# kakaoenterprise/JORLDY

Hardware: NVIDIA H100
Metric: env_steps_per_sec (higher is better)
Workload: dtype f32

## Files before the change

include/jorldy_b200.h:

```cpp
#ifndef JORLDY_B200_H
#define JORLDY_B200_H

#include <stdint.h>

#ifdef __cplusplus
#define JB_API extern "C"
#else
#define JB_API
#endif

JB_API int jb_env_classic_reset(int kind, double* phys, float* obs, int32_t* elapsed, int64_t* episode,
                                float* score, const uint8_t* mask, uint64_t seed, uint64_t stream_base,
                                int n, void* stream);
JB_API int jb_env_classic_step(int kind, double* phys, float* obs, int32_t* elapsed, int64_t* episode,
                               float* score, const void* action, int action_kind, float* next_obs,
                               float* reward, float* done, float* stats, int auto_reset, int max_steps,
                               uint64_t seed, uint64_t stream_base, int n, void* stream);

JB_API int jb_gae(const float* reward, const float* done, const float* value, const float* next_value,
                  const float* last_value, int N, int T, float gamma, float lambda, int standardize,
                  float* adv, float* ret, void* stream);

JB_API int
jb_env_synth_reset(float* obs, int32_t* elapsed, int64_t* episode, float* score, uint64_t seed,
// ... 59 lines not shown
JB_API int jb_heads_bwd_dw(const float* dout, const float* h, int M, int H, float* dw0, float* db0, int n0, float* dw1,
                           float* db1, int n1, float* dw2, float* db2, int n2, void* stream);
JB_API int jb_heads_fwd_n(const float* h, int M, int H, int n_heads, const float* const* w, const float* const* b,
                          const int* n, float* out, void* stream);
JB_API int jb_heads_bwd_dx_n(const float* dout, const float* h, int M, int H, int n_heads, const float* const* w,
                             const int* n, float* dh, void* stream);
JB_API int jb_heads_bwd_dw_n(const float* dout, const float* h, int M, int H, int n_heads, float* const* dw,
                             float* const* db, const int* n, void* stream);

JB_API int jb_ppo_act_discrete(const float* out, int M, int A, int nout, const float* u, uint64_t seed,
                               uint64_t stream_base, uint64_t ctr, long long* row_ctr, int greedy, int64_t* action,
                               void* stream);
JB_API int jb_ppo_act_continuous(const float* out, int M, int A, int nout, const float* normal, uint64_t seed,
                                 uint64_t stream_base, uint64_t ctr, long long* row_ctr, int greedy, float* action,
                                 void* stream);
JB_API int jb_ppo_prepass_discrete(const float* out, const int32_t* action, int M, int A, int nout, float* value,
                                   float* logp_old, void* stream);
JB_API int jb_ppo_prepass_continuous(const float* out, const float* action, int M, int A, int nout, float* value,
                                     float* logp_old, void* stream);
JB_API int jb_take_minibatch(const int32_t* perm, long long* cursor, int B, int32_t* cur_idx, void* stream);
JB_API int jb_ppo_loss(int continuous, const float* out, const int32_t* idx, const void* action, const float* adv,
                       const float* ret, const float* value_old, const float* logp_old, int B, int A, int nout,
                       float eps_clip, float vf_coef, float ent_coef, float* dout, float* stats, float* acc,
                       void* stream);

JB_API int jb_vmpo_loss(int continuous, const float* out, const float* out_old, const int32_t* idx, const void* action,
                        const float* adv, const float* ret, int B, int A, int nout, const float* mult, float eps_eta,
                        float eps_alpha_mu, float eps_alpha_sigma, float* dout, float* dmult, float* stats, float* acc,
                        void* stream);
JB_API int jb_vmpo_clamp(float* mult, float min_eta, float min_alpha_mu, float min_alpha_sigma, void* stream);
// ... 161 lines not shown
```

jorldy_b200/core/agent/ppo.py:

```python
import numpy as np
import torch

from ..buffer import FrameRollout, RolloutBuffer
from ..dev import C, ptr, require_cuda, stream_ptr
from ..network import Network
from ..optimizer import Optimizer
from .base import BaseAgent

GRAPH_CHUNK = 16
MAX_ACTION_SIZE = {"discrete": 18, "continuous": 8}


class PPO(BaseAgent):
    def __init__(
        self,
        state_size,
        action_size,
        hidden_size=512,
        network="discrete_policy_value",
        head="mlp",
        optim_config={"name": "adam"},
        gamma=0.99,
        use_standardization=True,
        run_step=1e6,
# ... 50 lines not shown
        self.use_fused = use_fused
        self._fused = {}
        self._graphs = {}
        self._acc = torch.zeros(8, dtype=torch.float32, device=self.device)
        self._cursor = torch.zeros(1, dtype=torch.int64, device=self.device)
        self.world_size = 1
        self.allreduce = None
        self._inject_perms = None
        self.n_launches = 0
        self.n_prepass_launches = 0

    @property
    def continuous(self):
        return self.action_type == "continuous"

    def act_device(self, state, training=True, noise=None):
        net = self.network
        M = state.shape[0]
        out = net._buf("act.out", (M, net.nout))
        net.forward_rows(state, out)
        A = self.action_size
        row_ctr = self._row_counter(M)
        if self.continuous:
            action = net._buf("act.a", (M, A))
            C.jb_ppo_act_continuous(ptr(out), M, A, net.nout, ptr(noise), self.seed, self.rng_stream_base,
                                    0, ptr(row_ctr), int(not training), ptr(action), stream_ptr())
        else:
            action = net._buf("act.a", (M,), torch.int64)
            C.jb_ppo_act_discrete(ptr(out), M, A, net.nout, ptr(noise), self.seed, self.rng_stream_base,
                                  0, ptr(row_ctr), int(not training), ptr(action), stream_ptr())
        return action

    @torch.no_grad()
    def act(self, state, training=True):
        self.network.train(training)
        s = self.as_tensor(state)
        action = self.act_device(s.view(s.shape[0], -1), training)
        a = action.cpu().numpy()
        return {"action": a.reshape(a.shape[0], -1)}

    def _minibatch_step(self, st, idx, B):
        net = self.network
        tag = f"mb{B}."
        out = net.forward_raw(st["state"], idx, B, tag=tag)
        dout = net._buf(tag + "dout", (B, net.nout))
# ... 43 lines not shown
            dst.copy_(src)
        graph = torch.cuda.CUDAGraph()
        with torch.cuda.graph(graph):
            chunk()
        self._graphs[key] = graph
        return graph

    def _gae_reward(self, st, reward, next_state, N, T):
        return reward

    def _advantages(self, st, state, action, reward, done, next_state, last_next_state, next_rows, N, T):
        net = self.network
        NT = N * T
        A = self.action_size
        s = stream_ptr()
        net.forward_rows(state, st["out"])
        if self.continuous:
            C.jb_ppo_prepass_continuous(ptr(st["out"]), ptr(action), NT, A, net.nout, ptr(st["value"]),
                                        ptr(st["logp_old"]), s)
        else:
            C.jb_ppo_prepass_discrete(ptr(st["out"]), ptr(action), NT, A, net.nout, ptr(st["value"]),
                                      ptr(st["logp_old"]), s)
        if next_state is not None:
            nout = net._buf("next.out", (NT, net.nout))
            net.forward_rows(next_state, nout)
            st["next_value"].copy_(nout[:, -1])
            nv, lv = st["next_value"], None
        else:
            lout = net._buf("last.out", (N, net.nout))
            net.forward_rows(last_next_state, lout)
            lv = net._buf("last.v", (N,))
            lv.copy_(lout[:, -1])
            nv = None
        reward = self._gae_reward(st, reward, next_state if next_state is not None else next_rows, N, T)
        C.jb_gae(ptr(reward), ptr(done), ptr(st["value"]), ptr(nv), ptr(lv), N, T, self.gamma, self._lambda,
                 int(self.use_standardization), ptr(st["adv"]), ptr(st["ret"]), s)
        return st["ret"].mean()

    def _learn_tensors(self, state, action, reward, done, next_state=None, last_next_state=None, next_rows=None):
        net = self.network
        NT = state.shape[0]
        T = self.n_step
        N = NT // T
        assert N * T == NT, f"rollout of {NT} rows is not a multiple of n_step={T} (ppo.py:97 view(-1, n_step) would raise)"
        A = self.action_size
        dev = self.device
        st = getattr(self, "_st", None)
        if st is None or st["NT"] != NT:
            st = {"NT": NT,
                  "out": torch.empty(NT, net.nout, device=dev),
                  "value": torch.empty(NT, device=dev),
                  "logp_old": torch.empty(NT, A if self.continuous else 1, device=dev),
                  "adv": torch.empty(NT, device=dev), "ret": torch.empty(NT, device=dev),
                  "next_value": torch.empty(NT, device=dev),
                  "perm": torch.empty(NT, dtype=torch.int32, device=dev)}
            self._st = st
        st["state"] = state
        st["action"] = action
        mean_ret = self._advantages(st, state, action, reward, done, next_state, last_next_state, next_rows, N, T)

        B = self.batch_size
        self._begin_epochs()
        n_full = NT // B
        tail = NT - n_full * B
        from . import ppo_fused
        use_fused = self.use_fused and n_full > 0 and ppo_fused.supported(self, B)
        if use_fused and B not in self._fused:
            self._fused[B] = ppo_fused.FusedRunner(self, B)
        use_graph = (not use_fused) and self.use_cuda_graph and n_full >= GRAPH_CHUNK
        n_steps = 0
        for epoch in range(self.n_epoch):
            if self._inject_perms is not None:
                perm = torch.as_tensor(np.asarray(self._inject_perms[epoch]), dtype=torch.int32, device=dev)
# ... 5 lines not shown
            if use_fused:
                self._fused[B].run(st, n_full)
                done_steps = n_full
            if use_graph:
                g = self._graph_for(st, B)
                for _ in range(n_full // GRAPH_CHUNK):
                    g.replay()
                done_steps = (n_full // GRAPH_CHUNK) * GRAPH_CHUNK
            for k in range(done_steps, n_full):
                self._minibatch_step(st, st["perm"][k * B:(k + 1) * B], B)
            if tail:
                self._minibatch_step(st, st["perm"][n_full * B:], tail)
            n_steps += n_full + (1 if tail else 0)
        self.n_launches = (self.n_epoch * (1 + (self.LAUNCHES_PER_MINIBATCH if tail else 0)) if use_fused
                           else n_steps * self.LAUNCHES_PER_MINIBATCH)
        n_chunks = (NT + 16383) // 16384
        self.n_prepass_launches = 3 * n_chunks + 1 + 3 + 1
        return self._learn_result(mean_ret)

    def _learn_result(self, mean_ret):
        acc = torch.cat([self._acc[:6], mean_ret.view(1), self._acc[7:8]]).cpu().numpy()
        if acc[7] != 0.0:
            dbg = [ws["partials"][200:205].tolist() for ws in (r.ws for r in self._fused.values())]
            raise RuntimeError("persistent PPO kernel: a peer GPU did not reach the gradient exchange (flag wait timed out); "
                               f"[kind 1=grad-ready 2=done-reading, peer, step, seen, target] = {dbg}")
        cnt = max(acc[5], 1.0)
        return {
            "actor_loss": float(acc[0] / cnt),
            "critic_loss": float(acc[1] / cnt),
            "entropy_loss": float(acc[2] / cnt),
            "max_ratio": float(acc[3]),
# ... 25 lines not shown
        hin["next_state"].copy_(torch.as_tensor(tr["next_state"], dtype=torch.float32, device=dev).reshape(n, -1))
        hin["reward"].copy_(torch.as_tensor(tr["reward"], dtype=torch.float32, device=dev).reshape(-1))
        hin["done"].copy_(torch.as_tensor(tr["done"], dtype=torch.float32, device=dev).reshape(-1))
        hin["action"].copy_(self._action_to_device(tr["action"]))
        return self._learn_tensors(hin["state"], hin["action"], hin["reward"], hin["done"], next_state=hin["next_state"])

    def learn_rollout(self, rollout):
        N, T = rollout.N, rollout.T
        frames = isinstance(rollout, FrameRollout)
        if frames:
            state, last = rollout.rows(), rollout.last_rows()
        else:
            state, last = rollout.state.view(N * T, -1), rollout.last_next_state
        res = self._learn_tensors(state, rollout.action.view(N * T, -1) if self.continuous
                                  else rollout.action.view(N * T), rollout.reward.view(N * T),
                                  rollout.done.view(N * T), last_next_state=last, next_rows=rollout.next_rows())
        if frames:
            rollout.frames.check()
        rollout.clear()
        return res

    def process(self, transitions, step):
        result = {}
        self.memory.store(transitions)
        delta_t = step - self.time_t
        self.time_t = step
        self.learn_stamp += delta_t
        if self.learn_stamp >= self.n_step:
            result = self.learn()
            if self.lr_decay:
                self.learning_rate_decay(step)
# ... 3 lines not shown
```

jorldy_b200/core/agent/rnd_ppo.py:

```python
import os

import numpy as np
import torch

from ..dev import C, ptr, stream_ptr
from ..network.policy_value import ContinuousPolicyTwoValue, DiscretePolicyTwoValue
from ..network.rnd import FEATURE, RND
from ..optimizer import Optimizer
from .base import cpu_state_dict
from .curiosity import _RunningMeanStd, check_batch_norm_rows, load_two_adam_state, two_adam_state
from .ppo import MAX_ACTION_SIZE, PPO

RND_NETWORKS = {"rnd_mlp": "mlp", "rnd_cnn": "cnn"}
TWO_VALUE_NETWORKS = {"discrete_policy_value": DiscretePolicyTwoValue, "continuous_policy_value": ContinuousPolicyTwoValue}


class RND_PPO(PPO):
    _GRAPH_INPUTS = PPO._GRAPH_INPUTS + ("value_i", "ret_i", "rnd_next", "rnd_target")
    replicas_only = True
    FAMILY = "RND-PPO"
    needs_next_state = True

    def __init__(self, state_size, action_size, optim_config={"name": "adam"}, rnd_network="rnd_mlp", gamma_i=0.99,
                 extrinsic_coeff=2.0, intrinsic_coeff=1.0, obs_normalize=True, ri_normalize=True, batch_norm=True,
# ... 62 lines not shown

    def _advantages(self, st, state, action, reward, done, next_state, last_next_state, next_rows, N, T):
        net = self.network
        NT = N * T
        s = stream_ptr()
        self._check_batch(NT)
        s_next = next_state if next_state is not None else next_rows
        if s_next is None:
            raise ValueError("RND-PPO needs every step's next state (a rollout with next_state, or host transitions)")
        st["rnd_next"] = s_next
        ri = self._intrinsic_reward(s_next, N, T)
        st["rnd_target"] = self.rnd.target_cache(NT)
        self._ri_mean = ri.mean()
        buf = lambda k: net._buf("rnd." + k, (NT,))
        st["value_i"], st["ret_i"] = buf("value_i"), buf("ret_i")
        net.forward_rows(state, st["out"])
        C.jb_rnd_prepass(int(self.continuous), ptr(st["out"]), ptr(action), NT, self.action_size, net.nout,
                         ptr(st["value"]), ptr(st["value_i"]), ptr(st["logp_old"]), s)
        nout = net._buf("next.out", (NT, net.nout))
        net.forward_rows(s_next, nout)
        st["next_value"].copy_(nout[:, -2])
        nv_i = buf("next_value_i")
        nv_i.copy_(nout[:, -1])
        adv_e, adv_i = buf("adv_e"), buf("adv_i")
        C.jb_gae(ptr(reward), ptr(done), ptr(st["value"]), ptr(st["next_value"]), 0, N, T, self.gamma, self._lambda, 0,
                 ptr(adv_e), ptr(st["ret"]), s)
        if self.non_episodic:
            done_i = buf("no_done")
            done_i.zero_()
        else:
# ... 75 lines not shown
```

jorldy_b200/core/buffer/rollout_buffer.py:

```python
import numpy as np
import torch

from ..dev import require_cuda
from .base import BaseBuffer
from .frame_store import FrameRows, FrameStore, frames_per_rollout


class RolloutBuffer(BaseBuffer):
    def __init__(self):
        super().__init__()
        self.buffer = list()

    def store(self, transitions):
        if self.first_store:
            self.check_dim(transitions[0])
        self.buffer += transitions

    def sample(self):
        transitions = self.stack_transition(self.buffer)
        self.buffer.clear()
        return transitions

    def sample_batched(self):
        out = {}
        for key in self.buffer[0].keys():
            arr = np.stack([np.asarray(b[key]) for b in self.buffer], axis=1)
            out[key] = arr.reshape((-1,) + arr.shape[2:])
        self.buffer.clear()
        return out

    @property
    def size(self):
        return len(self.buffer)


class DeviceRollout:

    def __init__(self, num_envs, n_step, state_size, action_size, action_type, device=None, next_state=False):
        dev = require_cuda(device)
        N, T = num_envs, n_step
        self.N, self.T, self.device = N, T, dev
        self.state = torch.zeros(N, T, state_size, dtype=torch.float32, device=dev)
        if action_type == "discrete":
            self.action = torch.zeros(N, T, dtype=torch.int32, device=dev)
        else:
            self.action = torch.zeros(N, T, action_size, dtype=torch.float32, device=dev)
        self.reward = torch.zeros(N, T, dtype=torch.float32, device=dev)
        self.done = torch.zeros(N, T, dtype=torch.float32, device=dev)
        self.last_next_state = torch.zeros(N, state_size, dtype=torch.float32, device=dev)
        self.next_state = torch.zeros(N, T, state_size, dtype=torch.float32, device=dev) if next_state else None
        self.t = 0

    def next_rows(self):
        return None if self.next_state is None else self.next_state.view(self.N * self.T, -1)

    def write(self, state, action, reward, done, next_state):
        t = self.t
        self.state[:, t].copy_(state)
        if self.action.dtype == torch.int32:
            self.action[:, t].copy_(action.view(self.N))
        else:
            self.action[:, t].copy_(action.view(self.N, -1))
        self.reward[:, t].copy_(reward)
        self.done[:, t].copy_(done)
        if self.next_state is not None:
            self.next_state[:, t].copy_(next_state)
        if t == self.T - 1:
            self.last_next_state.copy_(next_state)
        self.t = t + 1

    def write_after_step(self, action, reward, done, next_state):
        t = self.t
        if self.action.dtype == torch.int32:
            self.action[:, t].copy_(action.view(self.N))
        else:
            self.action[:, t].copy_(action.view(self.N, -1))
        self.reward[:, t].copy_(reward)
        self.done[:, t].copy_(done)
        if self.next_state is not None:
            self.next_state[:, t].copy_(next_state)
        if t == self.T - 1:
            self.last_next_state.copy_(next_state)
        self.t = t + 1

    @property
    def full(self):
        return self.t >= self.T

    def clear(self):
        self.t = 0

# ... 2 lines not shown

    def __init__(self, num_envs, n_step, action_size, action_type, device=None, next_state=False):
        dev = require_cuda(device)
        N, T = num_envs, n_step
        self.N, self.T, self.device = N, T, dev
        self.frames = FrameStore(N, frames_per_rollout(T), dev)
        self.state_ref = torch.zeros(N, T, dtype=torch.int64, device=dev)
        if action_type == "discrete":
            self.action = torch.zeros(N, T, dtype=torch.int32, device=dev)
        else:
            self.action = torch.zeros(N, T, action_size, dtype=torch.float32, device=dev)
        self.reward = torch.zeros(N, T, dtype=torch.float32, device=dev)
        self.done = torch.zeros(N, T, dtype=torch.float32, device=dev)
        self.last_next_state = torch.zeros(N, dtype=torch.int64, device=dev)
        self.next_state = None
        self.next_ref = torch.zeros(N, T, dtype=torch.int64, device=dev) if next_state else None
        self._refs = torch.zeros(2, N, dtype=torch.int64, device=dev)
        self.t = 0

    def start(self, obs):
        self.frames.start(obs)

    def push(self, obs, next_obs, done, auto_reset):
        s, x = self.frames.push(obs, next_obs, done, auto_reset, out=self._refs)
        self.state_ref[:, self.t].copy_(s)
        if self.next_ref is not None:
            self.next_ref[:, self.t].copy_(x)
        return x

    def rows(self):
# ... 8 lines not shown
```

jorldy_b200/core/collect.py:

```python
import torch

from .buffer import DeviceRollout, FrameRollout, frame_store


class RolloutCollector:
    def __init__(self, env, agent, n_step=None, use_cuda_graph=True):
        self.env, self.agent = env, agent
        self.T = n_step or agent.n_step
        self.frames = bool(getattr(env, "frame_stack", False))
        if self.frames:
            self.rollout = FrameRollout(env.num_envs, self.T, env.action_size, env.action_type, device=agent.device,
                                        next_state=getattr(agent, "needs_next_state", False))
        else:
            self.rollout = DeviceRollout(env.num_envs, self.T, env.state_size, env.action_size, env.action_type,
                                         device=agent.device, next_state=getattr(agent, "needs_next_state", False))
        self.use_cuda_graph = use_cuda_graph
        self._graph = None
        self.launches_per_collect = 5 * self.T
        env.reset_device()
        if self.frames:
            self.rollout.start(env.obs)

    def _collect_eager(self):
        env, agent, ro = self.env, self.agent, self.rollout
        ro.clear()
        for t in range(self.T):
            if not self.frames:
                ro.state[:, t].copy_(env.obs)
            action = agent.act_device(env.obs, training=True)
            next_obs, reward, done = env.step_device(action)
            ro.t = t
            if self.frames:
                next_obs = ro.push(env.obs, next_obs, done, env.auto_reset)
            ro.write_after_step(action, reward, done, next_obs)

    def collect(self):
        if not self.use_cuda_graph:
            self._collect_eager()
            return self.rollout
        if self._graph is None:
            side = torch.cuda.Stream()
            side.wait_stream(torch.cuda.current_stream())
            with torch.cuda.stream(side):
                self._collect_eager()
            torch.cuda.current_stream().wait_stream(side)
            torch.cuda.synchronize()
            g = torch.cuda.CUDAGraph()
            with torch.cuda.graph(g):
                self._collect_eager()
# ... 139 lines not shown
```

jorldy_b200/core/network/layers.py:

```python
from ..dev import C, ptr, stream_ptr


import ctypes
import os

TC_MIN_ROWS = 1024
_USE_TC = os.environ.get("JB_NO_TC", "0") != "1"


def linear_fwd(x, w, b, y, relu):
    M, in_f = x.shape
    out_f = w.shape[0]
    if _USE_TC and M >= TC_MIN_ROWS and M % 128 == 0 and out_f % 128 == 0 and in_f % 32 == 0 and b is not None:
        C.jb_linear_fwd_tc(ptr(x), ptr(w), ptr(b), ptr(y), M, in_f, out_f, int(relu), stream_ptr())
        return
    C.jb_linear_fwd(ptr(x), ptr(w), ptr(b), ptr(y), M, in_f, out_f, int(relu), stream_ptr())


def linear_bwd_dx(dy, w, dx, relu_act=None, accumulate=False):
    M, out_f = dy.shape
    in_f = w.shape[1]
    if accumulate:
        C.jb_gemm(ptr(dy), out_f, 1, ptr(w), in_f, 0, ptr(dx), in_f, M, in_f, out_f, 0, 0,
                  ptr(relu_act), in_f, 0, 1, stream_ptr())
# ... 25 lines not shown
    M, out_f = dy.shape
    C.jb_linear_io_bwd_dw(ptr(dy), ptr(x), ptr(dw), M, x.shape[1], out_f, stream_ptr())
    C.jb_colsum(ptr(dy), M, out_f, ptr(db), 0, stream_ptr())


def _ptrs(ts, kind=ctypes.c_void_p):
    return (kind * len(ts))(*ts)


def heads_fwd(h, heads, out):
    M, H = h.shape
    C.jb_heads_fwd_n(ptr(h), M, H, len(heads), _ptrs([ptr(w) for w, _ in heads]), _ptrs([ptr(b) for _, b in heads]),
                     _ptrs([w.shape[0] for w, _ in heads], ctypes.c_int), ptr(out), stream_ptr())


def heads_bwd_dx(dout, h, heads, dh):
    M, H = h.shape
    C.jb_heads_bwd_dx_n(ptr(dout), ptr(h), M, H, len(heads), _ptrs([ptr(w) for w, _ in heads]),
                        _ptrs([w.shape[0] for w, _ in heads], ctypes.c_int), ptr(dh), stream_ptr())


def heads_bwd_dw(dout, h, grads):
    M, H = h.shape
    C.jb_heads_bwd_dw_n(ptr(dout), ptr(h), M, H, len(grads), _ptrs([ptr(dw) for dw, _ in grads]),
                        _ptrs([ptr(db) for _, db in grads]), _ptrs([dw.shape[0] for dw, _ in grads], ctypes.c_int),
                        stream_ptr())
```

jorldy_b200/core/network/policy_value.py:

```python
import torch

from .base import FlatNetwork, init_gain, orthogonal_
from .head import make_head
from . import layers as L


class _PolicyValue(FlatNetwork):
    head_names = ()

    def __init__(self, D_in, D_out, D_hidden=512, head="mlp", device=None, seed=None):
        super().__init__(device)
        self.D_in, self.D_out, self.D_hidden = D_in, D_out, D_hidden
        self.head = make_head(head, D_in, D_hidden)
        self.out_heads = self._out_heads(D_out)
        self.nout = sum(n for _, n, _ in self.out_heads)
        self._wide = self.nout > 32
        assert not self._wide or len(self.out_heads) == 1
        specs = self.head.specs() + [("l.weight", (D_hidden, self.head.D_head_out)), ("l.bias", (D_hidden,))]
        for name, n, _ in self.out_heads:
            specs += [(f"{name}.weight", (n, D_hidden)), (f"{name}.bias", (n,))]
        self._specs = specs
        self._allocate()
        gen = torch.Generator().manual_seed(seed) if seed is not None else None
        with torch.no_grad():
            self.head.init(self.p, gen)
            self.p["l.weight"].copy_(orthogonal_((D_hidden, self.head.D_head_out), init_gain("relu"), gen))
            for name, n, gain in self.out_heads:
                self.p[f"{name}.weight"].copy_(orthogonal_((n, D_hidden), init_gain(gain), gen))

    def _heads_wb(self):
        return [(self.p[f"{n}.weight"], self.p[f"{n}.bias"]) for n, _, _ in self.out_heads]

    def _heads_grads(self):
        return [(self.g[f"{n}.weight"], self.g[f"{n}.bias"]) for n, _, _ in self.out_heads]

    def forward_raw(self, x, idx=None, M=None, out=None, tag="t.", save=True):
        M = M if M is not None else (idx.shape[0] if idx is not None else x.shape[0])
        h1 = self.head.forward(self, x, idx, M, tag, save)
        h2 = self._buf(tag + "h2", (M, self.D_hidden))
        L.linear_fwd(h1, self.p["l.weight"], self.p["l.bias"], h2, relu=True)
        if out is None:
            out = self._buf(tag + "out", (M, self.nout))
        if self._wide:
            w, b = self._heads_wb()[0]
            L.linear_fwd(h2, w, b, out, relu=False)
        else:
            L.heads_fwd(h2, self._heads_wb(), out)
        return out

    def forward_rows(self, x, out):
        M = x.shape[0]
        for s in range(0, M, self.head.max_rows):
            e = min(M, s + self.head.max_rows)
            self.forward_raw(x[s:e], None, e - s, out[s:e], tag=f"inf{e - s}.", save=False)
        return out

    def backward_raw(self, dout, M, tag="t."):
        h1 = self._buf(tag + "head.h", (M, self.head.D_head_out))
        h2 = self._buf(tag + "h2", (M, self.D_hidden))
        dh2 = self._buf(tag + "dh2", (M, self.D_hidden))
        dh1 = self._buf(tag + "dh1", (M, self.head.D_head_out))
        if self._wide:
            (w, _), (dw, db) = self._heads_wb()[0], self._heads_grads()[0]
            L.linear_bwd_dw(dout, h2, dw, db)
            L.linear_bwd_dx(dout, w, dh2, relu_act=h2)
        else:
            L.heads_bwd_dw(dout, h2, self._heads_grads())
            L.heads_bwd_dx(dout, h2, self._heads_wb(), dh2)
        L.linear_bwd_dw(dh2, h1, self.g["l.weight"], self.g["l.bias"])
# ... 37 lines not shown
```

jorldy_b200/csrc/heads.cu:

```cuda
#include "common.cuh"

namespace {

constexpr int MAX_DIN = 32;
constexpr int MAX_NOUT = 32;

__global__ void mlp_in_fwd_kernel(const float* __restrict__ x, const int32_t* __restrict__ idx,
                                  const float* __restrict__ W1, const float* __restrict__ b1,
                                  int M, int D, int H, float* __restrict__ h1, float* __restrict__ xg) {
  const int m = blockIdx.y;
  const int j = blockIdx.x * blockDim.x + threadIdx.x;
  __shared__ float sx[MAX_DIN];
  const int row = idx ? idx[m] : m;
  if (threadIdx.x < D) {
    const float v = x[(size_t)row * D + threadIdx.x];
    sx[threadIdx.x] = v;
    if (xg && blockIdx.x == 0) xg[(size_t)m * D + threadIdx.x] = v;
  }
  __syncthreads();
  if (j >= H) return;
  float acc = 0.f;
  for (int i = 0; i < D; ++i) acc = fmaf(sx[i], W1[(size_t)j * D + i], acc);
  acc += b1[j];
  h1[(size_t)m * H + j] = fmaxf(acc, 0.f);
}

struct HeadRows {
  const float* w[MAX_NOUT];
  const float* b[MAX_NOUT];
};
struct HeadGradRows {
  float* dw[MAX_NOUT];
  float* db[MAX_NOUT];
};

__global__ void __launch_bounds__(256)
heads_fwd_kernel(const float* __restrict__ h, int M, int H, HeadRows hr, int nout, float* __restrict__ out) {
  const int warp = (blockIdx.x * blockDim.x + threadIdx.x) >> 5;
  const int lane = threadIdx.x & 31;
  if (warp >= M) return;
  float acc[MAX_NOUT];
#pragma unroll
  for (int o = 0; o < MAX_NOUT; ++o) acc[o] = 0.f;
  const float* hrow = h + (size_t)warp * H;
  int j = lane;
  for (; j + 96 < H; j += 128) {
    float hv[4];
#pragma unroll
    for (int u = 0; u < 4; ++u) hv[u] = hrow[j + 32 * u];
#pragma unroll
    for (int o = 0; o < MAX_NOUT; ++o) {
      if (o < nout) {
        float wv[4];
#pragma unroll
        for (int u = 0; u < 4; ++u) wv[u] = hr.w[o][j + 32 * u];
#pragma unroll
        for (int u = 0; u < 4; ++u) acc[o] = fmaf(hv[u], wv[u], acc[o]);
      }
    }
  }
  for (; j < H; j += 32) {
    const float hv = hrow[j];
#pragma unroll
    for (int o = 0; o < MAX_NOUT; ++o)
      if (o < nout) acc[o] = fmaf(hv, hr.w[o][j], acc[o]);
  }
#pragma unroll
  for (int o = 0; o < MAX_NOUT; ++o) {
    if (o < nout) {
      const float v = jb_warp_sum(acc[o]);
      if (lane == 0) out[(size_t)warp * nout + o] = v + *hr.b[o];
    }
  }
}

__global__ void heads_bwd_dx_kernel(const float* __restrict__ dout, const float* __restrict__ h, int M, int H,
                                    HeadRows hr, int nout, float* __restrict__ dh) {
  const int m = blockIdx.y;
  const int j = blockIdx.x * blockDim.x + threadIdx.x;
  __shared__ float sd[MAX_NOUT];
  if (threadIdx.x < nout) sd[threadIdx.x] = dout[(size_t)m * nout + threadIdx.x];
  __syncthreads();
  if (j >= H) return;
  float acc = 0.f;
#pragma unroll
  for (int o = 0; o < MAX_NOUT; ++o)
    if (o < nout) acc = fmaf(sd[o], hr.w[o][j], acc);
  dh[(size_t)m * H + j] = (h[(size_t)m * H + j] > 0.f) ? acc : 0.f;
// ... 44 lines not shown
    float v = bacc;
#pragma unroll
    for (int q = 0; q < MAX_NOUT; ++q) if (q == o && o < nout) v = acc[q];
    __syncthreads();
    s[ry][threadIdx.x] = v;
    __syncthreads();
    if (ry == 0) {
      float t = s[0][threadIdx.x];
      for (int r = 1; r < DW_ROWS; ++r) t += s[r][threadIdx.x];
      if (o < nout) { if (j < H) gr.dw[o][j] = t; }
      else if (do_b) *gr.db[threadIdx.x] = t;
    }
  }
}

constexpr int MAX_HEADS = 4;

static bool fill_rows(HeadRows& hr, int n_heads, const float* const* w, const float* const* b, const int* n, int H) {
  int o = 0;
  for (int g = 0; g < n_heads; ++g)
    for (int q = 0; q < n[g]; ++q, ++o) {
      if (o >= MAX_NOUT || !w[g]) return false;
      hr.w[o] = w[g] + (size_t)q * H;
      hr.b[o] = b && b[g] ? b[g] + q : nullptr;
    }
  for (; o < MAX_NOUT; ++o) { hr.w[o] = nullptr; hr.b[o] = nullptr; }
  return true;
}

static int total_outputs(int n_heads, const int* n) {
  if (n_heads <= 0 || n_heads > MAX_HEADS || !n) return -1;
  int nout = 0;
  for (int g = 0; g < n_heads; ++g) {
    if (n[g] < 0) return -1;
    nout += n[g];
  }
  return nout > 0 && nout <= MAX_NOUT ? nout : -1;
}

}

JB_API int jb_mlp_in_fwd(const float* x, const int32_t* idx, const float* w1, const float* b1, int M, int D, int H,
                         float* h1, float* xg, void* stream) {
  if (!x || !w1 || !b1 || !h1 || M <= 0 || D <= 0 || D > MAX_DIN || H <= 0) return JB_ERR_INVALID;
  dim3 grid(jb_div_up(H, 128), M);
  mlp_in_fwd_kernel<<<grid, 128, 0, (cudaStream_t)stream>>>(x, idx, w1, b1, M, D, H, h1, xg);
  return jb_check_launch();
}

JB_API int jb_heads_fwd_n(const float* h, int M, int H, int n_heads, const float* const* w, const float* const* b,
                          const int* n, float* out, void* stream) {
  const int nout = total_outputs(n_heads, n);
  if (!h || !out || !w || !b || M <= 0 || H <= 0 || nout < 0) return JB_ERR_INVALID;
  for (int g = 0; g < n_heads; ++g) if (n[g] > 0 && (!w[g] || !b[g])) return JB_ERR_INVALID;
  HeadRows hr;
  if (!fill_rows(hr, n_heads, w, b, n, H)) return JB_ERR_INVALID;
  const int threads = 256;
  heads_fwd_kernel<<<jb_div_up((long long)M * 32, threads), threads, 0, (cudaStream_t)stream>>>(h, M, H, hr, nout, out);
  return jb_check_launch();
}

JB_API int jb_heads_bwd_dx_n(const float* dout, const float* h, int M, int H, int n_heads, const float* const* w,
                             const int* n, float* dh, void* stream) {
  const int nout = total_outputs(n_heads, n);
  if (!dout || !h || !dh || !w || M <= 0 || H <= 0 || nout < 0) return JB_ERR_INVALID;
  HeadRows hr;
  if (!fill_rows(hr, n_heads, w, nullptr, n, H)) return JB_ERR_INVALID;
  dim3 grid(jb_div_up(H, 128), M);
  heads_bwd_dx_kernel<<<grid, 128, 0, (cudaStream_t)stream>>>(dout, h, M, H, hr, nout, dh);
  return jb_check_launch();
}

JB_API int jb_heads_bwd_dw_n(const float* dout, const float* h, int M, int H, int n_heads, float* const* dw,
// ... 34 lines not shown
```

jorldy_b200/csrc/ppo.cu:

```cuda
#include "common.cuh"
#include "philox.cuh"
#include "ppo_rowmath.cuh"

namespace {

using jbppo::MAX_A;
using jbppo::MAX_A_DISC;
using jbppo::log_softmax_row;
using jbppo::atanh_clamped;

template <int NA>
__global__ void ppo_act_discrete_kernel(const float* __restrict__ out, int M, int A, int nout,
                                        const float* __restrict__ u_in, uint64_t seed, uint64_t stream_base,
                                        uint64_t ctr, long long* __restrict__ row_ctr, int greedy,
                                        int64_t* __restrict__ action) {
  const int m = blockIdx.x * blockDim.x + threadIdx.x;
  if (m >= M) return;
  ctr = jb_next_row_ctr(row_ctr, m, ctr);
  float lg[NA], lsm[NA];
#pragma unroll
  for (int a = 0; a < NA; ++a) lg[a] = a < A ? out[(size_t)m * nout + a] : 0.f;
  log_softmax_row<NA>(lg, A, lsm);
  int pick = 0;
  if (greedy) {
    float best = expf(lsm[0]);
#pragma unroll
    for (int a = 1; a < NA; ++a) if (a < A) { const float p = expf(lsm[a]); if (p > best) { best = p; pick = a; } }
  } else {
    float u;
    if (u_in) u = u_in[m];
    else { jb_philox4 r = jb_philox(seed, stream_base + (uint64_t)m, ctr); u = jb_u01_float(r.x); }
    float tot = 0.f;
#pragma unroll
    for (int a = 0; a < NA; ++a) if (a < A) tot += expf(lsm[a]);
    const float target = u * tot;
    float c = 0.f;
    bool found = false;
    pick = A - 1;
#pragma unroll
    for (int a = 0; a < NA; ++a) if (a < A && !found) { c += expf(lsm[a]); if (target < c) { pick = a; found = true; } }
  }
  action[m] = pick;
}

__global__ void ppo_act_continuous_kernel(const float* __restrict__ out, int M, int A, int nout,
                                          const float* __restrict__ n_in, uint64_t seed, uint64_t stream_base,
                                          uint64_t ctr, long long* __restrict__ row_ctr, int greedy,
                                          float* __restrict__ action) {
  const int m = blockIdx.x * blockDim.x + threadIdx.x;
  if (m >= M) return;
  ctr = jb_next_row_ctr(row_ctr, m, ctr);
  for (int a = 0; a < A; a += 2) {
    float n0 = 0.f, n1 = 0.f;
    if (!greedy) {
      if (n_in) { n0 = n_in[(size_t)m * A + a]; if (a + 1 < A) n1 = n_in[(size_t)m * A + a + 1]; }
      else jb_normal_pair(seed, stream_base + (uint64_t)m, ctr * 8 + (uint64_t)(a >> 1), n0, n1);
    }
    for (int q = 0; q < 2 && a + q < A; ++q) {
      const float mu = fminf(fmaxf(out[(size_t)m * nout + a + q], -5.f), 5.f);
      const float sd = expf(tanhf(out[(size_t)m * nout + A + a + q]));
      const float z = greedy ? mu : fmaf(sd, q ? n1 : n0, mu);
      action[(size_t)m * A + a + q] = tanhf(z);
    }
  }
}

template <int NA>
__global__ void ppo_prepass_discrete_kernel(const float* __restrict__ out, const int32_t* __restrict__ action,
                                            int M, int A, int nout, float* __restrict__ value,
                                            float* __restrict__ logp_old) {
  const int m = blockIdx.x * blockDim.x + threadIdx.x;
  if (m >= M) return;
  logp_old[m] = jbppo::logp_discrete<NA>(out + (size_t)m * nout, A, action[m]);
  value[m] = out[(size_t)m * nout + A];
}

__global__ void ppo_prepass_continuous_kernel(const float* __restrict__ out, const float* __restrict__ action,
                                              int M, int A, int nout, float* __restrict__ value,
// ... 88 lines not shown
  const dim3 grid(jb_div_up(M, 128));
  cudaStream_t s = (cudaStream_t)stream;
  if (A <= MAX_A) ppo_act_discrete_kernel<MAX_A><<<grid, 128, 0, s>>>(out, M, A, nout, u, seed, stream_base, ctr, row_ctr, greedy, action);
  else ppo_act_discrete_kernel<MAX_A_DISC><<<grid, 128, 0, s>>>(out, M, A, nout, u, seed, stream_base, ctr, row_ctr, greedy, action);
  return jb_check_launch();
}

JB_API int jb_ppo_act_continuous(const float* out, int M, int A, int nout, const float* normal, uint64_t seed,
                                 uint64_t stream_base, uint64_t ctr, long long* row_ctr, int greedy, float* action,
                                 void* stream) {
  if (!out || !action || M <= 0 || A <= 0 || A > MAX_A || nout < 2 * A) return JB_ERR_INVALID;
  ppo_act_continuous_kernel<<<jb_div_up(M, 128), 128, 0, (cudaStream_t)stream>>>(out, M, A, nout, normal, seed, stream_base, ctr, row_ctr, greedy, action);
  return jb_check_launch();
}

JB_API int jb_ppo_prepass_discrete(const float* out, const int32_t* action, int M, int A, int nout, float* value,
                                   float* logp_old, void* stream) {
  if (!out || !action || !value || !logp_old || M <= 0 || A <= 0 || A > MAX_A_DISC || nout != A + 1) return JB_ERR_INVALID;
  const dim3 grid(jb_div_up(M, 128));
  cudaStream_t s = (cudaStream_t)stream;
  if (A <= MAX_A) ppo_prepass_discrete_kernel<MAX_A><<<grid, 128, 0, s>>>(out, action, M, A, nout, value, logp_old);
  else ppo_prepass_discrete_kernel<MAX_A_DISC><<<grid, 128, 0, s>>>(out, action, M, A, nout, value, logp_old);
  return jb_check_launch();
}

JB_API int jb_ppo_prepass_continuous(const float* out, const float* action, int M, int A, int nout, float* value,
                                     float* logp_old, void* stream) {
  if (!out || !action || !value || !logp_old || M <= 0 || A <= 0 || A > MAX_A || nout != 2 * A + 1) return JB_ERR_INVALID;
  ppo_prepass_continuous_kernel<<<jb_div_up(M, 128), 128, 0, (cudaStream_t)stream>>>(out, action, M, A, nout, value, logp_old);
  return jb_check_launch();
// ... 18 lines not shown
```

Measured before the change: 2.029 million.

## Fuse policy heads with action sampling and reuse rollout outputs in learn

```diff
diff --git a/include/jorldy_b200.h b/include/jorldy_b200.h
--- a/include/jorldy_b200.h
+++ b/include/jorldy_b200.h
@@ -97,6 +97,10 @@
 JB_API int jb_ppo_act_continuous(const float* out, int M, int A, int nout, const float* normal, uint64_t seed,
                                  uint64_t stream_base, uint64_t ctr, long long* row_ctr, int greedy, float* action,
                                  void* stream);
+JB_API int jb_ppo_heads_act(int continuous, const float* h, int M, int H, int n_heads, const float* const* w,
+                            const float* const* b, const int* n, int A, const float* noise, uint64_t seed,
+                            uint64_t stream_base, long long* row_ctr, int greedy, float* out, long long ld_out, void* action,
+                            void* keep_action, long long ld_keep, void* stream);
 JB_API int jb_ppo_prepass_discrete(const float* out, const int32_t* action, int M, int A, int nout, float* value,
                                    float* logp_old, void* stream);
 JB_API int jb_ppo_prepass_continuous(const float* out, const float* action, int M, int A, int nout, float* value,
diff --git a/jorldy_b200/core/agent/ppo.py b/jorldy_b200/core/agent/ppo.py
--- a/jorldy_b200/core/agent/ppo.py
+++ b/jorldy_b200/core/agent/ppo.py
@@ -4,6 +4,7 @@
 from ..buffer import FrameRollout, RolloutBuffer
 from ..dev import C, ptr, require_cuda, stream_ptr
 from ..network import Network
+from ..network import layers as L
 from ..optimizer import Optimizer
 from .base import BaseAgent
 
@@ -88,21 +89,17 @@
     def continuous(self):
         return self.action_type == "continuous"
 
-    def act_device(self, state, training=True, noise=None):
+    def act_device(self, state, training=True, noise=None, keep=None):
         net = self.network
         M = state.shape[0]
-        out = net._buf("act.out", (M, net.nout))
-        net.forward_rows(state, out)
         A = self.action_size
         row_ctr = self._row_counter(M)
-        if self.continuous:
-            action = net._buf("act.a", (M, A))
-            C.jb_ppo_act_continuous(ptr(out), M, A, net.nout, ptr(noise), self.seed, self.rng_stream_base,
-                                    0, ptr(row_ctr), int(not training), ptr(action), stream_ptr())
-        else:
-            action = net._buf("act.a", (M,), torch.int64)
-            C.jb_ppo_act_discrete(ptr(out), M, A, net.nout, ptr(noise), self.seed, self.rng_stream_base,
-                                  0, ptr(row_ctr), int(not training), ptr(action), stream_ptr())
+        out, keep_action = keep if keep is not None else (net._buf("act.out", (M, net.nout)), None)
+        action = net._buf("act.a", (M, A)) if self.continuous else net._buf("act.a", (M,), torch.int64)
+        for s, e, h2 in net.trunk_rows(state):
+            L.heads_act(self.continuous, h2, net._heads_wb(), A, None if noise is None else noise[s:e], self.seed,
+                        self.rng_stream_base + s, row_ctr[s:e], not training, out[s:e], action[s:e],
+                        None if keep_action is None else keep_action[s:e])
         return action
 
     @torch.no_grad()
@@ -176,7 +173,8 @@
         NT = N * T
         A = self.action_size
         s = stream_ptr()
-        net.forward_rows(state, st["out"])
+        if st["out"] is st["out_buf"]:
+            net.forward_rows(state, st["out"])
         if self.continuous:
             C.jb_ppo_prepass_continuous(ptr(st["out"]), ptr(action), NT, A, net.nout, ptr(st["value"]),
                                         ptr(st["logp_old"]), s)
@@ -199,7 +197,7 @@
                  int(self.use_standardization), ptr(st["adv"]), ptr(st["ret"]), s)
         return st["ret"].mean()
 
-    def _learn_tensors(self, state, action, reward, done, next_state=None, last_next_state=None, next_rows=None):
+    def _learn_tensors(self, state, action, reward, done, next_state=None, last_next_state=None, next_rows=None, out=None):
         net = self.network
         NT = state.shape[0]
         T = self.n_step
@@ -210,7 +208,7 @@
         st = getattr(self, "_st", None)
         if st is None or st["NT"] != NT:
             st = {"NT": NT,
-                  "out": torch.empty(NT, net.nout, device=dev),
+                  "out_buf": torch.empty(NT, net.nout, device=dev),
                   "value": torch.empty(NT, device=dev),
                   "logp_old": torch.empty(NT, A if self.continuous else 1, device=dev),
                   "adv": torch.empty(NT, device=dev), "ret": torch.empty(NT, device=dev),
@@ -219,6 +217,7 @@
             self._st = st
         st["state"] = state
         st["action"] = action
+        st["out"] = out if out is not None else st["out_buf"]
         mean_ret = self._advantages(st, state, action, reward, done, next_state, last_next_state, next_rows, N, T)
 
         B = self.batch_size
@@ -254,7 +253,7 @@
             n_steps += n_full + (1 if tail else 0)
         self.n_launches = (self.n_epoch * (1 + (self.LAUNCHES_PER_MINIBATCH if tail else 0)) if use_fused
                            else n_steps * self.LAUNCHES_PER_MINIBATCH)
-        n_chunks = (NT + 16383) // 16384
+        n_chunks = (NT + 16383) // 16384 if st["out"] is st["out_buf"] else 0
         self.n_prepass_launches = 3 * n_chunks + 1 + 3 + 1
         return self._learn_result(mean_ret)
 
@@ -310,7 +309,8 @@
             state, last = rollout.state.view(N * T, -1), rollout.last_next_state
         res = self._learn_tensors(state, rollout.action.view(N * T, -1) if self.continuous
                                   else rollout.action.view(N * T), rollout.reward.view(N * T),
-                                  rollout.done.view(N * T), last_next_state=last, next_rows=rollout.next_rows())
+                                  rollout.done.view(N * T), last_next_state=last, next_rows=rollout.next_rows(),
+                                  out=None if rollout.out is None else rollout.out.view(N * T, -1))
         if frames:
             rollout.frames.check()
         rollout.clear()
diff --git a/jorldy_b200/core/agent/rnd_ppo.py b/jorldy_b200/core/agent/rnd_ppo.py
--- a/jorldy_b200/core/agent/rnd_ppo.py
+++ b/jorldy_b200/core/agent/rnd_ppo.py
@@ -100,6 +100,7 @@
         self._ri_mean = ri.mean()
         buf = lambda k: net._buf("rnd." + k, (NT,))
         st["value_i"], st["ret_i"] = buf("value_i"), buf("ret_i")
+        st["out"] = st["out_buf"]
         net.forward_rows(state, st["out"])
         C.jb_rnd_prepass(int(self.continuous), ptr(st["out"]), ptr(action), NT, self.action_size, net.nout,
                          ptr(st["value"]), ptr(st["value_i"]), ptr(st["logp_old"]), s)
diff --git a/jorldy_b200/core/buffer/rollout_buffer.py b/jorldy_b200/core/buffer/rollout_buffer.py
--- a/jorldy_b200/core/buffer/rollout_buffer.py
+++ b/jorldy_b200/core/buffer/rollout_buffer.py
@@ -36,7 +36,7 @@
 
 class DeviceRollout:
 
-    def __init__(self, num_envs, n_step, state_size, action_size, action_type, device=None, next_state=False):
+    def __init__(self, num_envs, n_step, state_size, action_size, action_type, device=None, next_state=False, nout=None):
         dev = require_cuda(device)
         N, T = num_envs, n_step
         self.N, self.T, self.device = N, T, dev
@@ -49,6 +49,7 @@
         self.done = torch.zeros(N, T, dtype=torch.float32, device=dev)
         self.last_next_state = torch.zeros(N, state_size, dtype=torch.float32, device=dev)
         self.next_state = torch.zeros(N, T, state_size, dtype=torch.float32, device=dev) if next_state else None
+        self.out = torch.zeros(N, T, nout, dtype=torch.float32, device=dev) if nout else None
         self.t = 0
 
     def next_rows(self):
@@ -71,10 +72,11 @@
 
     def write_after_step(self, action, reward, done, next_state):
         t = self.t
-        if self.action.dtype == torch.int32:
-            self.action[:, t].copy_(action.view(self.N))
-        else:
-            self.action[:, t].copy_(action.view(self.N, -1))
+        if action is not None:
+            if self.action.dtype == torch.int32:
+                self.action[:, t].copy_(action.view(self.N))
+            else:
+                self.action[:, t].copy_(action.view(self.N, -1))
         self.reward[:, t].copy_(reward)
         self.done[:, t].copy_(done)
         if self.next_state is not None:
@@ -107,6 +109,7 @@
         self.done = torch.zeros(N, T, dtype=torch.float32, device=dev)
         self.last_next_state = torch.zeros(N, dtype=torch.int64, device=dev)
         self.next_state = None
+        self.out = None
         self.next_ref = torch.zeros(N, T, dtype=torch.int64, device=dev) if next_state else None
         self._refs = torch.zeros(2, N, dtype=torch.int64, device=dev)
         self.t = 0
diff --git a/jorldy_b200/core/collect.py b/jorldy_b200/core/collect.py
--- a/jorldy_b200/core/collect.py
+++ b/jorldy_b200/core/collect.py
@@ -13,10 +13,11 @@
                                         next_state=getattr(agent, "needs_next_state", False))
         else:
             self.rollout = DeviceRollout(env.num_envs, self.T, env.state_size, env.action_size, env.action_type,
-                                         device=agent.device, next_state=getattr(agent, "needs_next_state", False))
+                                         device=agent.device, next_state=getattr(agent, "needs_next_state", False),
+                                         nout=agent.network.nout)
         self.use_cuda_graph = use_cuda_graph
         self._graph = None
-        self.launches_per_collect = 5 * self.T
+        self.launches_per_collect = 4 * self.T
         env.reset_device()
         if self.frames:
             self.rollout.start(env.obs)
@@ -25,14 +26,15 @@
         env, agent, ro = self.env, self.agent, self.rollout
         ro.clear()
         for t in range(self.T):
+            keep = None if self.frames else (ro.out[:, t], ro.action[:, t])
             if not self.frames:
                 ro.state[:, t].copy_(env.obs)
-            action = agent.act_device(env.obs, training=True)
+            action = agent.act_device(env.obs, training=True, keep=keep)
             next_obs, reward, done = env.step_device(action)
             ro.t = t
             if self.frames:
                 next_obs = ro.push(env.obs, next_obs, done, env.auto_reset)
-            ro.write_after_step(action, reward, done, next_obs)
+            ro.write_after_step(None if keep else action, reward, done, next_obs)
 
     def collect(self):
         if not self.use_cuda_graph:
diff --git a/jorldy_b200/core/network/layers.py b/jorldy_b200/core/network/layers.py
--- a/jorldy_b200/core/network/layers.py
+++ b/jorldy_b200/core/network/layers.py
@@ -63,6 +63,14 @@
                      _ptrs([w.shape[0] for w, _ in heads], ctypes.c_int), ptr(out), stream_ptr())
 
 
+def heads_act(continuous, h, heads, A, noise, seed, stream_base, row_ctr, greedy, out, action, keep_action=None):
+    M, H = h.shape
+    C.jb_ppo_heads_act(int(continuous), ptr(h), M, H, len(heads), _ptrs([ptr(w) for w, _ in heads]),
+                       _ptrs([ptr(b) for _, b in heads]), _ptrs([w.shape[0] for w, _ in heads], ctypes.c_int), A,
+                       ptr(noise), seed, stream_base, ptr(row_ctr), int(greedy), ptr(out), out.stride(0), ptr(action),
+                       ptr(keep_action), 0 if keep_action is None else keep_action.stride(0), stream_ptr())
+
+
 def heads_bwd_dx(dout, h, heads, dh):
     M, H = h.shape
     C.jb_heads_bwd_dx_n(ptr(dout), ptr(h), M, H, len(heads), _ptrs([ptr(w) for w, _ in heads]),
diff --git a/jorldy_b200/core/network/policy_value.py b/jorldy_b200/core/network/policy_value.py
--- a/jorldy_b200/core/network/policy_value.py
+++ b/jorldy_b200/core/network/policy_value.py
@@ -36,23 +36,34 @@
 
     def forward_raw(self, x, idx=None, M=None, out=None, tag="t.", save=True):
         M = M if M is not None else (idx.shape[0] if idx is not None else x.shape[0])
-        h1 = self.head.forward(self, x, idx, M, tag, save)
-        h2 = self._buf(tag + "h2", (M, self.D_hidden))
-        L.linear_fwd(h1, self.p["l.weight"], self.p["l.bias"], h2, relu=True)
+        h2 = self._trunk(x, idx, M, tag, save)
         if out is None:
             out = self._buf(tag + "out", (M, self.nout))
+        self._heads(h2, out)
+        return out
+
+    def _heads(self, h2, out):
         if self._wide:
             w, b = self._heads_wb()[0]
             L.linear_fwd(h2, w, b, out, relu=False)
         else:
             L.heads_fwd(h2, self._heads_wb(), out)
-        return out
 
-    def forward_rows(self, x, out):
+    def _trunk(self, x, idx, M, tag, save):
+        h1 = self.head.forward(self, x, idx, M, tag, save)
+        h2 = self._buf(tag + "h2", (M, self.D_hidden))
+        L.linear_fwd(h1, self.p["l.weight"], self.p["l.bias"], h2, relu=True)
+        return h2
+
+    def trunk_rows(self, x):
         M = x.shape[0]
         for s in range(0, M, self.head.max_rows):
             e = min(M, s + self.head.max_rows)
-            self.forward_raw(x[s:e], None, e - s, out[s:e], tag=f"inf{e - s}.", save=False)
+            yield s, e, self._trunk(x[s:e], None, e - s, f"inf{e - s}.", False)
+
+    def forward_rows(self, x, out):
+        for s, e, h2 in self.trunk_rows(x):
+            self._heads(h2, out[s:e])
         return out
 
     def backward_raw(self, dout, M, tag="t."):
diff --git a/jorldy_b200/csrc/heads.cu b/jorldy_b200/csrc/heads.cu
--- a/jorldy_b200/csrc/heads.cu
+++ b/jorldy_b200/csrc/heads.cu
@@ -1,9 +1,9 @@
 #include "common.cuh"
+#include "heads_row.cuh"
 
 namespace {
 
 constexpr int MAX_DIN = 32;
-constexpr int MAX_NOUT = 32;
 
 __global__ void mlp_in_fwd_kernel(const float* __restrict__ x, const int32_t* __restrict__ idx,
                                   const float* __restrict__ W1, const float* __restrict__ b1,
@@ -25,53 +25,23 @@
   h1[(size_t)m * H + j] = fmaxf(acc, 0.f);
 }
 
-struct HeadRows {
-  const float* w[MAX_NOUT];
-  const float* b[MAX_NOUT];
-};
+using jbheads::HeadRows;
+using jbheads::MAX_NOUT;
+using jbheads::fill_rows;
+using jbheads::total_outputs;
+
 struct HeadGradRows {
   float* dw[MAX_NOUT];
   float* db[MAX_NOUT];
 };
 
+template <int NB>
 __global__ void __launch_bounds__(256)
 heads_fwd_kernel(const float* __restrict__ h, int M, int H, HeadRows hr, int nout, float* __restrict__ out) {
   const int warp = (blockIdx.x * blockDim.x + threadIdx.x) >> 5;
   const int lane = threadIdx.x & 31;
   if (warp >= M) return;
-  float acc[MAX_NOUT];
-#pragma unroll
-  for (int o = 0; o < MAX_NOUT; ++o) acc[o] = 0.f;
-  const float* hrow = h + (size_t)warp * H;
-  int j = lane;
-  for (; j + 96 < H; j += 128) {
-    float hv[4];
-#pragma unroll
-    for (int u = 0; u < 4; ++u) hv[u] = hrow[j + 32 * u];
-#pragma unroll
-    for (int o = 0; o < MAX_NOUT; ++o) {
-      if (o < nout) {
-        float wv[4];
-#pragma unroll
-        for (int u = 0; u < 4; ++u) wv[u] = hr.w[o][j + 32 * u];
-#pragma unroll
-        for (int u = 0; u < 4; ++u) acc[o] = fmaf(hv[u], wv[u], acc[o]);
-      }
-    }
-  }
-  for (; j < H; j += 32) {
-    const float hv = hrow[j];
-#pragma unroll
-    for (int o = 0; o < MAX_NOUT; ++o)
-      if (o < nout) acc[o] = fmaf(hv, hr.w[o][j], acc[o]);
-  }
-#pragma unroll
-  for (int o = 0; o < MAX_NOUT; ++o) {
-    if (o < nout) {
-      const float v = jb_warp_sum(acc[o]);
-      if (lane == 0) out[(size_t)warp * nout + o] = v + *hr.b[o];
-    }
-  }
+  jbheads::row<NB>(h + (size_t)warp * H, H, hr, nout, lane, out + (size_t)warp * nout);
 }
 
 __global__ void heads_bwd_dx_kernel(const float* __restrict__ dout, const float* __restrict__ h, int M, int H,
@@ -146,30 +116,6 @@
   }
 }
 
-constexpr int MAX_HEADS = 4;
-
-static bool fill_rows(HeadRows& hr, int n_heads, const float* const* w, const float* const* b, const int* n, int H) {
-  int o = 0;
-  for (int g = 0; g < n_heads; ++g)
-    for (int q = 0; q < n[g]; ++q, ++o) {
-      if (o >= MAX_NOUT || !w[g]) return false;
-      hr.w[o] = w[g] + (size_t)q * H;
-      hr.b[o] = b && b[g] ? b[g] + q : nullptr;
-    }
-  for (; o < MAX_NOUT; ++o) { hr.w[o] = nullptr; hr.b[o] = nullptr; }
-  return true;
-}
-
-static int total_outputs(int n_heads, const int* n) {
-  if (n_heads <= 0 || n_heads > MAX_HEADS || !n) return -1;
-  int nout = 0;
-  for (int g = 0; g < n_heads; ++g) {
-    if (n[g] < 0) return -1;
-    nout += n[g];
-  }
-  return nout > 0 && nout <= MAX_NOUT ? nout : -1;
-}
-
 }
 
 JB_API int jb_mlp_in_fwd(const float* x, const int32_t* idx, const float* w1, const float* b1, int M, int D, int H,
@@ -187,8 +133,11 @@
   for (int g = 0; g < n_heads; ++g) if (n[g] > 0 && (!w[g] || !b[g])) return JB_ERR_INVALID;
   HeadRows hr;
   if (!fill_rows(hr, n_heads, w, b, n, H)) return JB_ERR_INVALID;
-  const int threads = 256;
-  heads_fwd_kernel<<<jb_div_up((long long)M * 32, threads), threads, 0, (cudaStream_t)stream>>>(h, M, H, hr, nout, out);
+  const int threads = 256, grid = jb_div_up((long long)M * 32, threads);
+  cudaStream_t s = (cudaStream_t)stream;
+  if (nout <= 4) heads_fwd_kernel<4><<<grid, threads, 0, s>>>(h, M, H, hr, nout, out);
+  else if (nout <= 8) heads_fwd_kernel<8><<<grid, threads, 0, s>>>(h, M, H, hr, nout, out);
+  else heads_fwd_kernel<MAX_NOUT><<<grid, threads, 0, s>>>(h, M, H, hr, nout, out);
   return jb_check_launch();
 }
 
diff --git a/jorldy_b200/csrc/heads_row.cuh b/jorldy_b200/csrc/heads_row.cuh
--- /dev/null
+++ b/jorldy_b200/csrc/heads_row.cuh
@@ -0,0 +1,74 @@
+#pragma once
+#include "common.cuh"
+
+namespace jbheads {
+
+constexpr int MAX_NOUT = 32;
+
+struct HeadRows {
+  const float* w[MAX_NOUT];
+  const float* b[MAX_NOUT];
+};
+
+template <int NB>
+__device__ __forceinline__ void row(const float* __restrict__ hrow, int H, const HeadRows& hr, int nout, int lane,
+                                    float* __restrict__ out_row) {
+  float acc[NB];
+#pragma unroll
+  for (int o = 0; o < NB; ++o) acc[o] = 0.f;
+  int j = lane;
+  for (; j + 96 < H; j += 128) {
+    float hv[4];
+#pragma unroll
+    for (int u = 0; u < 4; ++u) hv[u] = hrow[j + 32 * u];
+#pragma unroll
+    for (int o = 0; o < NB; ++o) {
+      if (o < nout) {
+        float wv[4];
+#pragma unroll
+        for (int u = 0; u < 4; ++u) wv[u] = hr.w[o][j + 32 * u];
+#pragma unroll
+        for (int u = 0; u < 4; ++u) acc[o] = fmaf(hv[u], wv[u], acc[o]);
+      }
+    }
+  }
+  for (; j < H; j += 32) {
+    const float hv = hrow[j];
+#pragma unroll
+    for (int o = 0; o < NB; ++o)
+      if (o < nout) acc[o] = fmaf(hv, hr.w[o][j], acc[o]);
+  }
+#pragma unroll
+  for (int o = 0; o < NB; ++o) {
+    if (o < nout) {
+      const float v = jb_warp_sum(acc[o]);
+      if (lane == 0) out_row[o] = v + *hr.b[o];
+    }
+  }
+}
+
+constexpr int MAX_HEADS = 4;
+
+inline bool fill_rows(HeadRows& hr, int n_heads, const float* const* w, const float* const* b, const int* n, int H) {
+  int o = 0;
+  for (int g = 0; g < n_heads; ++g)
+    for (int q = 0; q < n[g]; ++q, ++o) {
+      if (o >= MAX_NOUT || !w[g]) return false;
+      hr.w[o] = w[g] + (size_t)q * H;
+      hr.b[o] = b && b[g] ? b[g] + q : nullptr;
+    }
+  for (; o < MAX_NOUT; ++o) { hr.w[o] = nullptr; hr.b[o] = nullptr; }
+  return true;
+}
+
+inline int total_outputs(int n_heads, const int* n) {
+  if (n_heads <= 0 || n_heads > MAX_HEADS || !n) return -1;
+  int nout = 0;
+  for (int g = 0; g < n_heads; ++g) {
+    if (n[g] < 0) return -1;
+    nout += n[g];
+  }
+  return nout > 0 && nout <= MAX_NOUT ? nout : -1;
+}
+
+}
diff --git a/jorldy_b200/csrc/ppo.cu b/jorldy_b200/csrc/ppo.cu
--- a/jorldy_b200/csrc/ppo.cu
+++ b/jorldy_b200/csrc/ppo.cu
@@ -1,6 +1,7 @@
 #include "common.cuh"
 #include "philox.cuh"
 #include "ppo_rowmath.cuh"
+#include "heads_row.cuh"
 
 namespace {
 
@@ -8,6 +9,54 @@
 using jbppo::MAX_A_DISC;
 using jbppo::log_softmax_row;
 using jbppo::atanh_clamped;
+
+template <int NA>
+__device__ __forceinline__ int act_discrete_row(const float* o, int A, const float* u_in, uint64_t seed, uint64_t stream,
+                                                uint64_t ctr, int greedy) {
+  float lg[NA], lsm[NA];
+#pragma unroll
+  for (int a = 0; a < NA; ++a) lg[a] = a < A ? o[a] : 0.f;
+  log_softmax_row<NA>(lg, A, lsm);
+  int pick = 0;
+  if (greedy) {
+    float best = expf(lsm[0]);
+#pragma unroll
+    for (int a = 1; a < NA; ++a) if (a < A) { const float p = expf(lsm[a]); if (p > best) { best = p; pick = a; } }
+  } else {
+    float u;
+    if (u_in) u = *u_in;
+    else { jb_philox4 r = jb_philox(seed, stream, ctr); u = jb_u01_float(r.x); }
+    float tot = 0.f;
+#pragma unroll
+    for (int a = 0; a < NA; ++a) if (a < A) tot += expf(lsm[a]);
+    const float target = u * tot;
+    float c = 0.f;
+    bool found = false;
+    pick = A - 1;
+#pragma unroll
+    for (int a = 0; a < NA; ++a) if (a < A && !found) { c += expf(lsm[a]); if (target < c) { pick = a; found = true; } }
+  }
+  return pick;
+}
+
+__device__ __forceinline__ void act_continuous_row(const float* o, int A, const float* n_in, uint64_t seed, uint64_t stream,
+                                                   uint64_t ctr, int greedy, float* act, float* keep) {
+  for (int a = 0; a < A; a += 2) {
+    float n0 = 0.f, n1 = 0.f;
+    if (!greedy) {
+      if (n_in) { n0 = n_in[a]; if (a + 1 < A) n1 = n_in[a + 1]; }
+      else jb_normal_pair(seed, stream, ctr * 8 + (uint64_t)(a >> 1), n0, n1);
+    }
+    for (int q = 0; q < 2 && a + q < A; ++q) {
+      const float mu = fminf(fmaxf(o[a + q], -5.f), 5.f);
+      const float sd = expf(tanhf(o[A + a + q]));
+      const float z = greedy ? mu : fmaf(sd, q ? n1 : n0, mu);
+      const float v = tanhf(z);
+      act[a + q] = v;
+      if (keep) keep[a + q] = v;
+    }
+  }
+}
 
 template <int NA>
 __global__ void ppo_act_discrete_kernel(const float* __restrict__ out, int M, int A, int nout,
@@ -17,30 +66,8 @@
   const int m = blockIdx.x * blockDim.x + threadIdx.x;
   if (m >= M) return;
   ctr = jb_next_row_ctr(row_ctr, m, ctr);
-  float lg[NA], lsm[NA];
-#pragma unroll
-  for (int a = 0; a < NA; ++a) lg[a] = a < A ? out[(size_t)m * nout + a] : 0.f;
-  log_softmax_row<NA>(lg, A, lsm);
-  int pick = 0;
-  if (greedy) {
-    float best = expf(lsm[0]);
-#pragma unroll
-    for (int a = 1; a < NA; ++a) if (a < A) { const float p = expf(lsm[a]); if (p > best) { best = p; pick = a; } }
-  } else {
-    float u;
-    if (u_in) u = u_in[m];
-    else { jb_philox4 r = jb_philox(seed, stream_base + (uint64_t)m, ctr); u = jb_u01_float(r.x); }
-    float tot = 0.f;
-#pragma unroll
-    for (int a = 0; a < NA; ++a) if (a < A) tot += expf(lsm[a]);
-    const float target = u * tot;
-    float c = 0.f;
-    bool found = false;
-    pick = A - 1;
-#pragma unroll
-    for (int a = 0; a < NA; ++a) if (a < A && !found) { c += expf(lsm[a]); if (target < c) { pick = a; found = true; } }
-  }
-  action[m] = pick;
+  action[m] = act_discrete_row<NA>(out + (size_t)m * nout, A, u_in ? u_in + m : nullptr, seed, stream_base + (uint64_t)m,
+                                   ctr, greedy);
 }
 
 __global__ void ppo_act_continuous_kernel(const float* __restrict__ out, int M, int A, int nout,
@@ -50,18 +77,33 @@
   const int m = blockIdx.x * blockDim.x + threadIdx.x;
   if (m >= M) return;
   ctr = jb_next_row_ctr(row_ctr, m, ctr);
-  for (int a = 0; a < A; a += 2) {
-    float n0 = 0.f, n1 = 0.f;
-    if (!greedy) {
-      if (n_in) { n0 = n_in[(size_t)m * A + a]; if (a + 1 < A) n1 = n_in[(size_t)m * A + a + 1]; }
-      else jb_normal_pair(seed, stream_base + (uint64_t)m, ctr * 8 + (uint64_t)(a >> 1), n0, n1);
-    }
-    for (int q = 0; q < 2 && a + q < A; ++q) {
-      const float mu = fminf(fmaxf(out[(size_t)m * nout + a + q], -5.f), 5.f);
-      const float sd = expf(tanhf(out[(size_t)m * nout + A + a + q]));
-      const float z = greedy ? mu : fmaf(sd, q ? n1 : n0, mu);
-      action[(size_t)m * A + a + q] = tanhf(z);
-    }
+  act_continuous_row(out + (size_t)m * nout, A, n_in ? n_in + (size_t)m * A : nullptr, seed, stream_base + (uint64_t)m, ctr,
+                     greedy, action + (size_t)m * A, nullptr);
+}
+
+constexpr int HA_THREADS = 256;
+template <bool CONT, int NA, int NB>
+__global__ void __launch_bounds__(HA_THREADS)
+ppo_heads_act_kernel(const float* __restrict__ h, int M, int H, jbheads::HeadRows hr, int nout, int A,
+                     const float* __restrict__ noise, uint64_t seed, uint64_t stream_base, long long* __restrict__ row_ctr,
+                     int greedy, float* __restrict__ out, long long ld_out, void* __restrict__ action,
+                     void* __restrict__ keep_action, long long ld_keep) {
+  __shared__ float srow[HA_THREADS / 32][jbheads::MAX_NOUT];
+  const int m = (blockIdx.x * blockDim.x + threadIdx.x) >> 5;
+  const int lane = threadIdx.x & 31;
+  if (m >= M) return;
+  float* o = srow[threadIdx.x >> 5];
+  jbheads::row<NB>(h + (size_t)m * H, H, hr, nout, lane, o);
+  if (lane != 0) return;
+  for (int q = 0; q < nout; ++q) out[(size_t)m * ld_out + q] = o[q];
+  const uint64_t ctr = jb_next_row_ctr(row_ctr, m, 0);
+  if constexpr (CONT) {
+    act_continuous_row(o, A, noise ? noise + (size_t)m * A : nullptr, seed, stream_base + (uint64_t)m, ctr, greedy,
+                       (float*)action + (size_t)m * A, keep_action ? (float*)keep_action + (size_t)m * ld_keep : nullptr);
+  } else {
+    const int a = act_discrete_row<NA>(o, A, noise ? noise + m : nullptr, seed, stream_base + (uint64_t)m, ctr, greedy);
+    ((int64_t*)action)[m] = a;
+    if (keep_action) ((int32_t*)keep_action)[(size_t)m * ld_keep] = a;
   }
 }
 
@@ -180,6 +222,37 @@
   return jb_check_launch();
 }
 
+JB_API int jb_ppo_heads_act(int continuous, const float* h, int M, int H, int n_heads, const float* const* w,
+                            const float* const* b, const int* n, int A, const float* noise, uint64_t seed,
+                            uint64_t stream_base, long long* row_ctr, int greedy, float* out, long long ld_out, void* action,
+                            void* keep_action, long long ld_keep, void* stream) {
+  const int nout = jbheads::total_outputs(n_heads, n);
+  if (!h || !w || !b || !out || !action || M <= 0 || H <= 0 || nout < 0 || ld_out < nout) return JB_ERR_INVALID;
+  if (A <= 0 || A > (continuous ? MAX_A : MAX_A_DISC) || nout < (continuous ? 2 * A : A)) return JB_ERR_INVALID;
+  if (keep_action && ld_keep < (continuous ? A : 1)) return JB_ERR_INVALID;
+  for (int g = 0; g < n_heads; ++g) if (n[g] > 0 && (!w[g] || !b[g])) return JB_ERR_INVALID;
+  jbheads::HeadRows hr;
+  if (!jbheads::fill_rows(hr, n_heads, w, b, n, H)) return JB_ERR_INVALID;
+  const unsigned grid = (unsigned)jb_div_up((long long)M * 32, HA_THREADS);
+  cudaStream_t s = (cudaStream_t)stream;
+#define JB_HEADS_ACT(CONT, NA, NB)                                                                                    \
+  ppo_heads_act_kernel<CONT, NA, NB><<<grid, HA_THREADS, 0, s>>>(h, M, H, hr, nout, A, noise, seed, stream_base, row_ctr, \
+                                                                 greedy, out, ld_out, action, keep_action, ld_keep)
+  if (continuous) {
+    if (nout <= 4) JB_HEADS_ACT(true, MAX_A, 4);
+    else if (nout <= 8) JB_HEADS_ACT(true, MAX_A, 8);
+    else JB_HEADS_ACT(true, MAX_A, jbheads::MAX_NOUT);
+  } else if (A <= MAX_A) {
+    if (nout <= 4) JB_HEADS_ACT(false, MAX_A, 4);
+    else if (nout <= 8) JB_HEADS_ACT(false, MAX_A, 8);
+    else JB_HEADS_ACT(false, MAX_A, jbheads::MAX_NOUT);
+  } else {
+    JB_HEADS_ACT(false, MAX_A_DISC, jbheads::MAX_NOUT);
+  }
+#undef JB_HEADS_ACT
+  return jb_check_launch();
+}
+
 JB_API int jb_ppo_prepass_discrete(const float* out, const int32_t* action, int M, int A, int nout, float* value,
                                    float* logp_old, void* stream) {
   if (!out || !action || !value || !logp_old || M <= 0 || A <= 0 || A > MAX_A_DISC || nout != A + 1) return JB_ERR_INVALID;
```

Result: faster. 2.083 million, median of 6 (+2.7%).
